# lorenlugosch/end-to-end-SLU

Hardware: AMD Instinct MI355X
Metric: utterances/sec (train step, 3 s @16 kHz, B=64) (higher is better)
Workload: dtype f32 (trainable stages: exact fp32 MFMA; convolutions and GRU contractions of FROZEN stages: bf16x3 = every fp32 operand split EXACTLY into 3 bf16 terms (3 x 8 = 24 significand bits, fp32's exponent range), 6 bf16 MFMA products per fp32 product (only terms below 2^-24 |a b| dropped), fp32 accumulatio; 1 GPU; experiments/no_unfreezing.cfg SLU train step (frozen SincNet/conv/biGRU encoder in train mode + intent biGRU trained): fwd + 3-slot CE + bwd + grad all-reduce + Adam; batch_per_gpu=64, global_batch=64, samples_per_utterance=48000, parallelism=dp1, encoder_lookahead_batches=20

## Files before the change

end-to-end-slu_amd/csrc/slu_gru_bf16.hip:

```cpp
#include "slu_bf16.h"
#include <type_traits>

namespace slu {

__device__ __forceinline__ float bf_sigmoid(float x) {
  return __builtin_amdgcn_rcpf(1.0f + __builtin_amdgcn_exp2f(-1.4426950408889634f * x));
}
__device__ __forceinline__ float bf_tanh(float x) {
  return 1.0f - 2.0f * __builtin_amdgcn_rcpf(1.0f + __builtin_amdgcn_exp2f(2.8853900817779268f * x));
}

__device__ __forceinline__ void lds_barrier() { asm volatile("s_waitcnt lgkmcnt(0)\n\ts_barrier" ::: "memory"); }

__device__ __forceinline__ float mul_rnd(float a, float b) {
#pragma clang fp contract(off)
  return a * b;
}
__device__ __forceinline__ float add_rnd(float a, float b) {
#pragma clang fp contract(off)
  return a + b;
}

struct GruBfParams {
  const float* gx;
  const unsigned short* xp; long long x_plane;
  const uint4* wih; const float* b_ih;
  const float* w_hh[2];
  const float* b_hh[2];
  float* out;
  float* reserve;
  unsigned short* planes; long long plane;
  const unsigned* keep;
  float keep_scale;
  int T, B, D;
};

template <int H, int NS, int KI, int EPI>
struct GruLds {
  static constexpr int ROWB = H * 2;
  static constexpr int GXROW = 3 * H + 8;
  static constexpr int OROW = H + 4;
  static constexpr int PROWB = H * 2 + 16;
  static constexpr int HBUF = 2 * NS * 16 * ROWB;
  static constexpr int BIAS = KI > 0 ? 2 * 3 * H * 4 : 0;
  static constexpr int GXS = KI > 0 ? 0 : 2 * 16 * GXROW * 4;
  static constexpr int OST = EPI == 1 ? 2 * NS * 16 * PROWB : 2 * 16 * OROW * 4;
  static constexpr int BYTES = HBUF + BIAS + GXS + OST;
};

template <int H, int NS, int KI, int EPI, bool REV>
__device__ __forceinline__ void gru_bf_fwd_body(const GruBfParams& p) {
  constexpr int NW = H / 16;
  constexpr int KC = H / 32;
  constexpr int SLOTS = H / 8;
  constexpr bool BIAS_LDS = KI > 0;
  typedef Split<NS> SP;
  typedef GruLds<H, NS, KI, EPI> LD;
  constexpr int ROWB = LD::ROWB, GXROW = LD::GXROW, OROW = LD::OROW, PROWB = LD::PROWB;
  extern __shared__ __attribute__((aligned(16))) unsigned char smem[];
  unsigned char* const hbuf = smem;
  float* const bias_s = reinterpret_cast<float*>(smem + LD::HBUF);
  float* const gxs = reinterpret_cast<float*>(smem + LD::HBUF + LD::BIAS);
  unsigned char* const ost = smem + LD::HBUF + LD::BIAS + LD::GXS;
  const int tid = threadIdx.x, lane = tid & 63;
  const int w = __builtin_amdgcn_readfirstlane(tid >> 6);
  const int i = lane & 15, kg = lane >> 4;
  constexpr int dir = REV ? 1 : 0;
  const int b0 = blockIdx.x * 16;
  const int u0 = w * 16 + kg * 4;
  const int T = p.T, B = p.B, D = p.D;
  const int seq = b0 + i;
  const int seqc = seq < B ? seq : B - 1;

  if constexpr (NS == 2) f16_denorm_flush();

  uint4 wb[3][KC][NS];
  {
    const float* __restrict__ W = p.w_hh[dir];
#pragma unroll
    for (int g = 0; g < 3; ++g)
#pragma unroll
      for (int c = 0; c < KC; ++c) {
        const float* src = W + (size_t)(g * H + w * 16 + i) * H + c * 32 + kg * 8;
        const float4 lo = *reinterpret_cast<const float4*>(src), hi = *reinterpret_cast<const float4*>(src + 4);
        const float v[8] = {lo.x, lo.y, lo.z, lo.w, hi.x, hi.y, hi.z, hi.w};
        unsigned short s[8][NS];
#pragma unroll
        for (int e = 0; e < 8; ++e) split_terms<NS>(v[e], s[e]);
#pragma unroll
        for (int pl = 0; pl < NS; ++pl) {
          uint4 o;
          o.x = s[0][pl] | ((unsigned)s[1][pl] << 16); o.y = s[2][pl] | ((unsigned)s[3][pl] << 16);
          o.z = s[4][pl] | ((unsigned)s[5][pl] << 16); o.w = s[6][pl] | ((unsigned)s[7][pl] << 16);
          wb[g][c][pl] = o;
        }
      }
  }
  float bh[3][4];
  if constexpr (BIAS_LDS) {
    for (int x = tid; x < 3 * H; x += H * 4) {
      bias_s[x] = p.b_hh[dir][x];
      bias_s[3 * H + x] = p.b_ih[(size_t)dir * 3 * H + x];
    }
  } else {
#pragma unroll
    for (int g = 0; g < 3; ++g) {
      const float4 v = *reinterpret_cast<const float4*>(p.b_hh[dir] + g * H + u0);
      bh[g][0] = v.x; bh[g][1] = v.y; bh[g][2] = v.z; bh[g][3] = v.w;
    }
  }
  constexpr int KIA = KI > 0 ? KI : 1;
  uint4 wi[3][KIA][NS];
  if constexpr (KI > 0) {
    const int NTI = p.D * 3 * NW;
#pragma unroll
    for (int g = 0; g < 3; ++g)
#pragma unroll
      for (int c = 0; c < KI; ++c)
#pragma unroll
        for (int pl = 0; pl < NS; ++pl)
          wi[g][c][pl] = p.wih[(size_t)pl * KI * NTI * 64 + ((size_t)c * NTI + dir * 3 * NW + g * NW + w) * 64 + lane];
  }
  auto xproj = [&](const uint4 (&xa)[KIA][NS], float (&o)[3][4]) {
    f32x4 ax[SP::NACC][3];
#pragma unroll
    for (int a = 0; a < SP::NACC; ++a)
#pragma unroll
      for (int g = 0; g < 3; ++g) ax[a][g] = f32x4{0.f, 0.f, 0.f, 0.f};
#pragma unroll
    for (int c = 0; c < KIA; ++c)
#pragma unroll
      for (int q = 0; q < SP::NPAIR; ++q)
#pragma unroll
        for (int g = 0; g < 3; ++g)
          ax[SP::ACC(q)][g] = mfma_split<NS>(wi[g][c][SP::PB(q)], xa[c][SP::PA(q)], ax[SP::ACC(q)][g]);
#pragma unroll
    for (int g = 0; g < 3; ++g) {
      const f32x4 v = split_result<NS>(ax[0][g], ax[SP::NACC - 1][g]);
      const float4 bi = *reinterpret_cast<const float4*>(&bias_s[BIAS_LDS ? 3 * H + g * H + u0 : 0]);
      o[g][0] = v[0] + bi.x; o[g][1] = v[1] + bi.y; o[g][2] = v[2] + bi.z; o[g][3] = v[3] + bi.w;
    }
  };
  auto xload = [&](int t_, uint4 (&xa)[KIA][NS]) {
    const unsigned short* base = p.xp + ((size_t)t_ * B + seqc) * (32 * KIA) + kg * 8;
#pragma unroll
    for (int c = 0; c < KIA; ++c)
#pragma unroll
      for (int pl = 0; pl < NS; ++pl)
        xa[c][pl] = *reinterpret_cast<const uint4*>(base + (size_t)pl * p.x_plane + c * 32);
  };

  constexpr int RW = 16 / NW;
  constexpr int GLR = 3 * H / 4;
  auto gx_g = [&](int j) { const int f = j * 64 + lane; return min(b0 + RW * w + f / GLR, B - 1) * D * 3 * H + dir * 3 * H + (f % GLR) * 4; };
  auto gx_s = [&](int j) { const int f = j * 64 + lane; return (RW * w + f / GLR) * GXROW + (f % GLR) * 4; };
  const int gx_g0 = gx_g(0), gx_g1 = gx_g(1), gx_g2 = gx_g(2);
  const int gx_s0 = gx_s(0), gx_s1 = gx_s(1), gx_s2 = gx_s(2);
  const size_t gx_ts = (size_t)B * D * 3 * H, out_ts = (size_t)B * D * H;
#define SLU_GX_REQUEST(t_, a, b, c)                                                         \
  do {                                                                                      \
    const float* gp__ = p.gx + (size_t)(t_) * gx_ts;                                        \
    a = *reinterpret_cast<const float4*>(gp__ + gx_g0);                                     \
    b = *reinterpret_cast<const float4*>(gp__ + gx_g1);                                     \
    c = *reinterpret_cast<const float4*>(gp__ + gx_g2);                                     \
  } while (0)
#define SLU_GX_STAGE(buf, a, b, c)                                                          \
  do {                                                                                      \
    float* gs__ = gxs + (buf) * (16 * GXROW);                                               \
    *reinterpret_cast<float4*>(gs__ + gx_s0) = a;                                           \
    *reinterpret_cast<float4*>(gs__ + gx_s1) = b;                                           \
    *reinterpret_cast<float4*>(gs__ + gx_s2) = c;                                           \
  } while (0)
  const int orow = RW * w + lane / (H / 4), oc16 = lane % (H / 4);
  const bool orow_ok = b0 + orow < B;
  const int o_goff = (b0 + orow) * D * H + dir * H + oc16 * 4;

  int a_off[KC];
#pragma unroll
  for (int c = 0; c < KC; ++c) a_off[c] = i * ROWB + (((c * 4 + kg) ^ i) & (SLOTS - 1)) * 16;
  const int h_off = i * ROWB + ((((u0 >> 3) ^ i) & (SLOTS - 1)) * 16) + (u0 & 7) * 2;
  const int gs_off = i * GXROW + u0;
  const int os_off = i * OROW + u0;
  const int ps_off = i * PROWB + u0 * 2;
  const int kw_off = seqc * ((D * H) >> 5) + ((dir * H + u0) >> 5);
  const int kw_sh = (dir * H + u0) & 31;
  const size_t kw_ts = (size_t)B * ((D * H) >> 5);
  const bool drop = EPI > 0 && p.keep != nullptr;

  for (int x = tid; x < 2 * NS * 16 * ROWB / 4; x += H * 4) reinterpret_cast<unsigned*>(hbuf)[x] = 0u;
  float hprev[4] = {0.f, 0.f, 0.f, 0.f};
  float gcur[3][4];
  unsigned kcur = 0;
  {
    const int t0 = dir ? T - 1 : 0;
    if constexpr (KI > 0) {
      __syncthreads();
      uint4 xa0[KIA][NS];
      xload(t0, xa0);
      xproj(xa0, gcur);
    } else {
      float4 ga, gb, gc;
      SLU_GX_REQUEST(t0, ga, gb, gc);
      SLU_GX_STAGE(0, ga, gb, gc);
    }
    if (drop) kcur = p.keep[(size_t)t0 * kw_ts + kw_off];
  }
  float held[4] = {0.f, 0.f, 0.f, 0.f};
  int pend_t = -1;
  int pend_buf = 0;
  auto flush = [&]() {
    if (pend_t < 0) return;
    if constexpr (EPI == 1) {
      constexpr int LPR = H / 8;
      constexpr int NCH = NS * 16 * LPR / 64;
      for (int c = w; c < NCH; c += NW) {
        const int f = c * 64 + lane, pl = f / (16 * LPR), r = (f / LPR) % 16, c16 = f % LPR;
        if (b0 + r < B) {
          const uint4 v = *reinterpret_cast<const uint4*>(ost + ((pend_buf * NS + pl) * 16 + r) * PROWB + c16 * 16);
          *reinterpret_cast<uint4*>(p.planes + (size_t)pl * p.plane + (size_t)pend_t * out_ts + (b0 + r) * D * H + dir * H + c16 * 8) = v;
        }
      }
    } else {
      if (orow_ok) {
        const float4 v = *reinterpret_cast<const float4*>(reinterpret_cast<const float*>(ost) + (pend_buf * 16 + orow) * OROW + oc16 * 4);
        *reinterpret_cast<float4*>(p.out + (size_t)pend_t * out_ts + o_goff) = v;
      }
    }
  };
  __syncthreads();
  __builtin_amdgcn_s_waitcnt(0x0F70);

  auto step = [&](auto cur_c, const int s) {
    constexpr int cur = decltype(cur_c)::value;
    const int t = dir ? T - 1 - s : s;
    const int tn = (s + 1 < T) ? (dir ? t - 1 : t + 1) : t;

    if constexpr (BIAS_LDS) {
#pragma unroll
      for (int g = 0; g < 3; ++g) {
        const float4 v = *reinterpret_cast<const float4*>(&bias_s[g * H + u0]);
        bh[g][0] = v.x; bh[g][1] = v.y; bh[g][2] = v.z; bh[g][3] = v.w;
      }
    }
    if constexpr (KI == 0) {
#pragma unroll
      for (int g = 0; g < 3; ++g) {
        const float4 v = *reinterpret_cast<const float4*>(gxs + cur * (16 * GXROW) + gs_off + g * H);
        gcur[g][0] = v.x; gcur[g][1] = v.y; gcur[g][2] = v.z; gcur[g][3] = v.w;
      }
    }
    f32x4 accs[SP::NACC][3];
#pragma unroll
    for (int a = 0; a < SP::NACC; ++a)
#pragma unroll
      for (int g = 0; g < 3; ++g) accs[a][g] = f32x4{0.f, 0.f, 0.f, 0.f};
    float gn[4];
#pragma unroll
    for (int r = 0; r < 4; ++r) {
      accs[0][0][r] = gcur[0][r] + bh[0][r];
      accs[0][1][r] = gcur[1][r] + bh[1][r];
      accs[0][2][r] = bh[2][r];
      gn[r] = gcur[2][r];
    }
    const unsigned kbits = kcur >> kw_sh;

    float gnext[3][4];
    float4 gl0 = make_float4(0.f, 0.f, 0.f, 0.f), gl1 = gl0, gl2 = gl0;
    uint4 xan[KIA][NS];
    if constexpr (KI > 0) xload(tn, xan);
    else SLU_GX_REQUEST(tn, gl0, gl1, gl2);
    unsigned knext = 0;
    if (drop) knext = p.keep[(size_t)tn * kw_ts + kw_off];
    flush();

    const unsigned char* hc = hbuf + cur * (NS * 16 * ROWB);
    float hn[4];
#pragma unroll
    for (int c = 0; c < KC; ++c) {
      uint4 fa[NS];
#pragma unroll
      for (int pl = 0; pl < NS; ++pl) fa[pl] = *reinterpret_cast<const uint4*>(hc + pl * (16 * ROWB) + a_off[c]);
#pragma unroll
      for (int q = 0; q < SP::NPAIR; ++q)
#pragma unroll
        for (int g = 0; g < 3; ++g)
          accs[SP::ACC(q)][g] = mfma_split<NS>(wb[g][c][SP::PB(q)], fa[SP::PA(q)], accs[SP::ACC(q)][g]);
    }
    f32x4 acc[3];
#pragma unroll
    for (int g = 0; g < 3; ++g) acc[g] = split_result<NS>(accs[0][g], accs[SP::NACC - 1][g]);

#pragma unroll
    for (int r = 0; r < 4; ++r) {
      const float rr = bf_sigmoid(acc[0][r]);
      const float zz = bf_sigmoid(acc[1][r]);
      const float nn = bf_tanh(gn[r] + rr * acc[2][r]);
      hn[r] = nn + zz * (hprev[r] - nn);
    }
    {
      unsigned char* __restrict__ hnext = hbuf + (cur ^ 1) * (NS * 16 * ROWB);
      if constexpr (NS == 2) {
        unsigned hi01, lo01, hi23, lo23;
        split_f16x2_pair_flush(hn[0], hn[1], hi01, lo01);
        split_f16x2_pair_flush(hn[2], hn[3], hi23, lo23);
        *reinterpret_cast<uint2*>(hnext + h_off) = make_uint2(hi01, hi23);
        *reinterpret_cast<uint2*>(hnext + 16 * ROWB + h_off) = make_uint2(lo01, lo23);
      } else if constexpr (NS == 3) {
        unsigned w01[3], w23[3];
        split_bf16x3_pair(hn[0], hn[1], w01);
        split_bf16x3_pair(hn[2], hn[3], w23);
#pragma unroll
        for (int pl = 0; pl < 3; ++pl)
          *reinterpret_cast<uint2*>(hnext + pl * (16 * ROWB) + h_off) = make_uint2(w01[pl], w23[pl]);
      } else {
        unsigned short sp[4][NS];
#pragma unroll
        for (int r = 0; r < 4; ++r) split_terms<NS>(hn[r], sp[r]);
#pragma unroll
        for (int pl = 0; pl < NS; ++pl)
          *reinterpret_cast<uint2*>(hnext + pl * (16 * ROWB) + h_off) =
              make_uint2(sp[0][pl] | ((unsigned)sp[1][pl] << 16), sp[2][pl] | ((unsigned)sp[3][pl] << 16));
      }
    }
    if constexpr (EPI == 0) {
      *reinterpret_cast<float4*>(reinterpret_cast<float*>(ost) + cur * (16 * OROW) + os_off) = make_float4(hn[0], hn[1], hn[2], hn[3]);
      pend_t = t; pend_buf = cur;
    } else {
      float m[4];
#pragma unroll
      for (int r = 0; r < 4; ++r)
        m[r] = drop ? mul_rnd(hn[r], ((kbits >> r) & 1u) ? p.keep_scale : 0.0f) : hn[r];
      const bool even = dir ? (t & 1) == 0 : cur == 0;
      const bool single = even && t == T - 1;
      const bool emit = dir ? even : (!even || single);
      pend_t = -1;
      if (!emit) {
#pragma unroll
        for (int r = 0; r < 4; ++r) held[r] = dir ? m[r] : add_rnd(0.0f, m[r]);
      } else {
        float v[4];
#pragma unroll
        for (int r = 0; r < 4; ++r) {
          const float first = dir ? add_rnd(0.0f, m[r]) : held[r];
          const float second = dir ? held[r] : m[r];
          v[r] = mul_rnd(add_rnd(first, second), 0.5f);
        }
        if (single) {
          asm volatile("" ::: "memory");
#pragma unroll
          for (int r = 0; r < 4; ++r) v[r] = add_rnd(0.0f, m[r]);
        }
        pend_t = t >> 1; pend_buf = cur;
        if constexpr (EPI == 2) {
          *reinterpret_cast<float4*>(reinterpret_cast<float*>(ost) + cur * (16 * OROW) + os_off) = make_float4(v[0], v[1], v[2], v[3]);
        } else if constexpr (NS == 2) {
          unsigned hi01, lo01, hi23, lo23;
          split_f16x2_pair_flush(v[0], v[1], hi01, lo01);
          split_f16x2_pair_flush(v[2], v[3], hi23, lo23);
          *reinterpret_cast<uint2*>(ost + ((cur * NS + 0) * 16) * PROWB + ps_off) = make_uint2(hi01, hi23);
          *reinterpret_cast<uint2*>(ost + ((cur * NS + 1) * 16) * PROWB + ps_off) = make_uint2(lo01, lo23);
        } else if constexpr (NS == 3) {
          unsigned w01[3], w23[3];
          split_bf16x3_pair(v[0], v[1], w01);
          split_bf16x3_pair(v[2], v[3], w23);
#pragma unroll
          for (int pl = 0; pl < 3; ++pl)
            *reinterpret_cast<uint2*>(ost + ((cur * NS + pl) * 16) * PROWB + ps_off) = make_uint2(w01[pl], w23[pl]);
        } else {
          unsigned short sp[4][NS];
#pragma unroll
          for (int r = 0; r < 4; ++r) split_terms<NS>(v[r], sp[r]);
#pragma unroll
          for (int pl = 0; pl < NS; ++pl)
            *reinterpret_cast<uint2*>(ost + ((cur * NS + pl) * 16) * PROWB + ps_off) =
                make_uint2(sp[0][pl] | ((unsigned)sp[1][pl] << 16), sp[2][pl] | ((unsigned)sp[3][pl] << 16));
        }
      }
    }
    if constexpr (KI > 0) {
      xproj(xan, gnext);
#pragma unroll
      for (int g = 0; g < 3; ++g)
#pragma unroll
        for (int r = 0; r < 4; ++r) gcur[g][r] = gnext[g][r];
    } else {
      SLU_GX_STAGE(cur ^ 1, gl0, gl1, gl2);
    }
#pragma unroll
    for (int r = 0; r < 4; ++r) hprev[r] = hn[r];
    kcur = knext;
    lds_barrier();
  };
  {
    int s = 0;
    for (; s + 1 < T; s += 2) {
      step(std::integral_constant<int, 0>{}, s);
      step(std::integral_constant<int, 1>{}, s + 1);
    }
    if (s < T) step(std::integral_constant<int, 0>{}, s);
  }
  flush();
#undef SLU_GX_REQUEST
#undef SLU_GX_STAGE
}

template <int H, int NS, int KI, int EPI>
__global__ void __launch_bounds__(H * 4)
gru_bf_fwd_kernel(const GruBfParams p) {
  if (blockIdx.y) gru_bf_fwd_body<H, NS, KI, EPI, true>(p);
  else gru_bf_fwd_body<H, NS, KI, EPI, false>(p);
}

template <int H, int NS, int EPI>
struct Gru2Lds {
  static constexpr int ROWB = H * 2;
  static constexpr int OROW = H + 4;
  static constexpr int PROWB = H * 2 + 16;
  static constexpr int HB = NS * 16 * ROWB;
  static constexpr int GXB = 16 * 3 * H * 4;
  static constexpr int KBB = 16 * (H / 32) * 4;
  static constexpr int OSB = EPI == 1 ? NS * 16 * PROWB : 16 * OROW * 4;
  static constexpr int HBUF = 0;
  static constexpr int GXR = HBUF + 2 * HB;
  static constexpr int KBR = GXR + 3 * GXB;
  static constexpr int BIAS = KBR + 3 * KBB;
  static constexpr int OST = BIAS + 3 * H * 4;
  static constexpr int HP = OST + 2 * OSB;
  static constexpr int HELD = HP + 2 * 16 * H * 4;
  static constexpr int BYTES = HELD + (EPI > 0 ? 2 * 16 * H * 4 : 0);
};

__device__ __forceinline__ void dma_b128(const void* base, unsigned voff, unsigned lds_addr) {
  asm volatile("s_mov_b32 m0, %2\n\ts_nop 0\n\tglobal_load_lds_dwordx4 %0, %1" :: "v"(voff), "s"(base), "s"(lds_addr) : "memory");
}
__device__ __forceinline__ void dma_b32(const void* base, unsigned voff, unsigned lds_addr) {
  asm volatile("s_mov_b32 m0, %2\n\ts_nop 0\n\tglobal_load_lds_dword %0, %1" :: "v"(voff), "s"(base), "s"(lds_addr) : "memory");
}

template <int H, int NS, int EPI>
__global__ void __launch_bounds__(H * 4)
gru_bf2_fwd_kernel(const GruBfParams p) {
  static_assert(H == 128, "two-tile recurrence: H = 128 (8 waves = two per SIMD, one keep-word DMA per chunk)");
  constexpr int NW = H / 16, KC = H / 32, SLOTS = H / 8;
  typedef Split<NS> SP;
  typedef Gru2Lds<H, NS, EPI> LD;
  constexpr int ROWB = LD::ROWB, OROW = LD::OROW, PROWB = LD::PROWB;
  constexpr int PCS = 3 * H / 4;
  extern __shared__ __attribute__((aligned(16))) unsigned char smem[];
  typedef __attribute__((address_space(3))) void* lptr_t;
  const unsigned lds0 = (unsigned)(size_t)(lptr_t)smem;
  float* const bias_s = reinterpret_cast<float*>(smem + LD::BIAS);
  const int tid = threadIdx.x, lane = tid & 63;
  const int w = __builtin_amdgcn_readfirstlane(tid >> 6);
  const int i = lane & 15, kg = lane >> 4;
  const int dir = blockIdx.y;
  const int b0 = blockIdx.x * 32;
  const int u0 = w * 16 + kg * 4;
  const int T = p.T, B = p.B, D = p.D;

  if constexpr (NS == 2) f16_denorm_flush();

  uint4 wb[3][KC][NS];
  {
    const float* __restrict__ W = p.w_hh[dir];
#pragma unroll
    for (int g = 0; g < 3; ++g)
#pragma unroll
      for (int c = 0; c < KC; ++c) {
        const float* src = W + (size_t)(g * H + w * 16 + i) * H + c * 32 + kg * 8;
        const float4 lo = *reinterpret_cast<const float4*>(src), hi = *reinterpret_cast<const float4*>(src + 4);
        const float v[8] = {lo.x, lo.y, lo.z, lo.w, hi.x, hi.y, hi.z, hi.w};
        unsigned short s[8][NS];
#pragma unroll
        for (int e = 0; e < 8; ++e) split_terms<NS>(v[e], s[e]);
#pragma unroll
        for (int pl = 0; pl < NS; ++pl) {
          uint4 o;
          o.x = s[0][pl] | ((unsigned)s[1][pl] << 16); o.y = s[2][pl] | ((unsigned)s[3][pl] << 16);
          o.z = s[4][pl] | ((unsigned)s[5][pl] << 16); o.w = s[6][pl] | ((unsigned)s[7][pl] << 16);
          wb[g][c][pl] = o;
        }
      }
  }
  for (int x = tid; x < 3 * H; x += H * 4) bias_s[x] = p.b_hh[dir][x];
  for (int x = tid; x < 2 * LD::HB / 4; x += H * 4) reinterpret_cast<unsigned*>(smem + LD::HBUF)[x] = 0u;
  __syncthreads();

  const bool drop = EPI > 0 && p.keep != nullptr;
  unsigned gv[2][3];
#pragma unroll
  for (int x = 0; x < 2; ++x)
#pragma unroll
    for (int j = 0; j < 3; ++j) {
      const int P = (3 * w + j) * 64 + lane, row = P / PCS, q = P % PCS;
      gv[x][j] = (unsigned)((min(b0 + 16 * x + row, B - 1) * D * 3 * H + dir * 3 * H) * 4 + (q ^ (row & 15)) * 16);
    }
  unsigned kv[2];
  const int KW = (D * H) >> 5;
#pragma unroll
  for (int x = 0; x < 2; ++x)
    kv[x] = drop ? (unsigned)((min(b0 + 16 * x + (lane >> 2), B - 1) * KW + dir * (H >> 5) + (lane & 3)) * 4) : (unsigned)(lane * 4);
  const void* const kbase = drop ? (const void*)p.keep : (const void*)p.gx;
  const size_t gx_ts = (size_t)B * D * 3 * H * 4, kw_ts = drop ? (size_t)B * KW * 4 : 0, out_ts = (size_t)B * D * H;
  const unsigned gx_m0 = lds0 + LD::GXR + 3 * w * 1024, kb_m0 = lds0 + LD::KBR;
  auto dma_chunk = [&](int x, int t_, int slot) {
    const char* gb = reinterpret_cast<const char*>(p.gx) + (size_t)t_ * gx_ts;
    const unsigned m = gx_m0 + slot * LD::GXB;
    const unsigned v0 = x ? gv[1][0] : gv[0][0], v1 = x ? gv[1][1] : gv[0][1], v2 = x ? gv[1][2] : gv[0][2];
    dma_b128(gb, v0, m);
    dma_b128(gb, v1, m + 1024);
    dma_b128(gb, v2, m + 2048);
    dma_b32(reinterpret_cast<const char*>(kbase) + (size_t)t_ * kw_ts, x ? kv[1] : kv[0], kb_m0 + slot * LD::KBB);
  };

  const int a_off0 = i * ROWB + ((kg ^ i) & (SLOTS - 1)) * 16;
  const int h_off = i * ROWB + ((((u0 >> 3) ^ i) & (SLOTS - 1)) * 16) + (u0 & 7) * 2;
  const int gs_off0 = (i * PCS + ((u0 >> 2) ^ i)) * 16;
  const int hp_off = (i * H + u0) * 4;
  const int kb_off = (i * (H >> 5) + (u0 >> 5)) * 4;
  const int kb_sh = u0 & 31;
  const int os_off = i * OROW + u0;
  const int ps_off = i * PROWB + u0 * 2;
  const int orow = (16 / NW) * w + lane / (H / 4), oc16 = lane % (H / 4);

  f32x4 accs[2][SP::NACC][3];
  float gn[2][4];
  unsigned kb[2] = {0u, 0u};
  int pend[2] = {-1, -1};
#pragma unroll
  for (int x = 0; x < 2; ++x) {
#pragma unroll
    for (int r = 0; r < 4; ++r) gn[x][r] = 0.f;
    *reinterpret_cast<float4*>(smem + LD::HP + x * (16 * H * 4) + hp_off) = make_float4(0.f, 0.f, 0.f, 0.f);
    if constexpr (EPI > 0) *reinterpret_cast<float4*>(smem + LD::HELD + x * (16 * H * 4) + hp_off) = make_float4(0.f, 0.f, 0.f, 0.f);
  }
#pragma unroll
  for (int x = 0; x < 2; ++x)
#pragma unroll
    for (int a = 0; a < SP::NACC; ++a)
#pragma unroll
      for (int g = 0; g < 3; ++g) accs[x][a][g] = f32x4{0.f, 0.f, 0.f, 0.f};

#define SLU_G2_M(X, slot)                                                                                              \
  do {                                                                                                                 \
    const unsigned char* gxc__ = smem + LD::GXR + (slot) * LD::GXB;                                                    \
    _Pragma("unroll") for (int g = 0; g < 3; ++g) {                                                                    \
      const float4 v = *reinterpret_cast<const float4*>(gxc__ + gs_off0 + g * (4 * H));                                \
      const float4 bb = *reinterpret_cast<const float4*>(&bias_s[g * H + u0]);                                         \
      _Pragma("unroll") for (int a = 0; a < SP::NACC; ++a) accs[X][a][g] = f32x4{0.f, 0.f, 0.f, 0.f};                  \
      if (g < 2) accs[X][0][g] = f32x4{v.x + bb.x, v.y + bb.y, v.z + bb.z, v.w + bb.w};                                \
      else { accs[X][0][g] = f32x4{bb.x, bb.y, bb.z, bb.w}; gn[X][0] = v.x; gn[X][1] = v.y; gn[X][2] = v.z; gn[X][3] = v.w; } \
    }                                                                                                                  \
    kb[X] = *reinterpret_cast<const unsigned*>(smem + LD::KBR + (slot) * LD::KBB + kb_off) >> kb_sh;                   \
    const unsigned char* hc__ = smem + LD::HBUF + (X) * LD::HB;                                                        \
    _Pragma("unroll") for (int c = 0; c < KC; ++c) {                                                                   \
      uint4 fa[NS];                                                                                                    \
      _Pragma("unroll") for (int pl = 0; pl < NS; ++pl) fa[pl] = *reinterpret_cast<const uint4*>(hc__ + pl * (16 * ROWB) + (a_off0 ^ (c * 64))); \
      _Pragma("unroll") for (int q = 0; q < SP::NPAIR; ++q)                                                            \
        _Pragma("unroll") for (int g = 0; g < 3; ++g)                                                                  \
          accs[X][SP::ACC(q)][g] = mfma_split<NS>(wb[g][c][SP::PB(q)], fa[SP::PA(q)], accs[X][SP::ACC(q)][g]);         \
    }                                                                                                                  \
  } while (0)

#define SLU_G2_G(X, t_)                                                                                                \
  do {                                                                                                                 \
    f32x4 acc[3];                                                                                                      \
    _Pragma("unroll") for (int g = 0; g < 3; ++g) acc[g] = split_result<NS>(accs[X][0][g], accs[X][SP::NACC - 1][g]);  \
    float hn[4];                                                                                                       \
    float4* const hp__ = reinterpret_cast<float4*>(smem + LD::HP + (X) * (16 * H * 4) + hp_off);                       \
    const float4 hpv = *hp__;                                                                                          \
    const float hprev[4] = {hpv.x, hpv.y, hpv.z, hpv.w};                                                               \
    _Pragma("unroll") for (int r = 0; r < 4; ++r) {                                                                    \
      const float rr = bf_sigmoid(acc[0][r]);                                                                          \
      const float zz = bf_sigmoid(acc[1][r]);                                                                          \
      const float nn = bf_tanh(gn[X][r] + rr * acc[2][r]);                                                             \
      hn[r] = nn + zz * (hprev[r] - nn);                                                                               \
    }                                                                                                                  \
    *hp__ = make_float4(hn[0], hn[1], hn[2], hn[3]);                                                                   \
    {                                                                                                                  \
      unsigned char* __restrict__ hx = smem + LD::HBUF + (X) * LD::HB;                                                 \
      if constexpr (NS == 2) {                                                                                         \
        unsigned hi01, lo01, hi23, lo23;                                                                               \
        split_f16x2_pair_flush(hn[0], hn[1], hi01, lo01);                                                              \
        split_f16x2_pair_flush(hn[2], hn[3], hi23, lo23);                                                              \
        *reinterpret_cast<uint2*>(hx + h_off) = make_uint2(hi01, hi23);                                                \
        *reinterpret_cast<uint2*>(hx + 16 * ROWB + h_off) = make_uint2(lo01, lo23);                                    \
      } else if constexpr (NS == 3) {                                                                                  \
        unsigned w01[3], w23[3];                                                                                       \
        split_bf16x3_pair(hn[0], hn[1], w01);                                                                          \
        split_bf16x3_pair(hn[2], hn[3], w23);                                                                          \
        _Pragma("unroll") for (int pl = 0; pl < 3; ++pl)                                                               \
          *reinterpret_cast<uint2*>(hx + pl * (16 * ROWB) + h_off) = make_uint2(w01[pl], w23[pl]);                     \
      } else {                                                                                                         \
        unsigned short sp[4][NS];                                                                                      \
        _Pragma("unroll") for (int r = 0; r < 4; ++r) split_terms<NS>(hn[r], sp[r]);                                   \
        _Pragma("unroll") for (int pl = 0; pl < NS; ++pl)                                                              \
          *reinterpret_cast<uint2*>(hx + pl * (16 * ROWB) + h_off) =                                                   \
              make_uint2(sp[0][pl] | ((unsigned)sp[1][pl] << 16), sp[2][pl] | ((unsigned)sp[3][pl] << 16));            \
      }                                                                                                                \
    }                                                                                                                  \
    unsigned char* const ox__ = smem + LD::OST + (X) * LD::OSB;                                                        \
    if constexpr (EPI == 0) {                                                                                          \
      *reinterpret_cast<float4*>(reinterpret_cast<float*>(ox__) + os_off) = make_float4(hn[0], hn[1], hn[2], hn[3]);   \
      pend[X] = (t_);                                                                                                  \
    } else {                                                                                                           \
      float m[4];                                                                                                      \
      _Pragma("unroll") for (int r = 0; r < 4; ++r)                                                                    \
        m[r] = drop ? __fmul_rn(hn[r], ((kb[X] >> r) & 1u) ? p.keep_scale : 0.0f) : hn[r];                             \
      const bool even = ((t_) & 1) == 0;                                                                               \
      const bool single = even && (t_) == T - 1;                                                                       \
      const bool emit = dir ? even : (!even || single);                                                                \
      pend[X] = -1;                                                                                                    \
      float4* const hl__ = reinterpret_cast<float4*>(smem + LD::HELD + (X) * (16 * H * 4) + hp_off);                   \
      if (!emit) {                                                                                                     \
        float hd[4];                                                                                                   \
        _Pragma("unroll") for (int r = 0; r < 4; ++r) hd[r] = dir ? m[r] : __fadd_rn(0.0f, m[r]);                      \
        *hl__ = make_float4(hd[0], hd[1], hd[2], hd[3]);                                                               \
      } else {                                                                                                         \
        const float4 hlv = *hl__;                                                                                      \
        const float held[4] = {hlv.x, hlv.y, hlv.z, hlv.w};                                                            \
        float v[4];                                                                                                    \
        _Pragma("unroll") for (int r = 0; r < 4; ++r) {                                                                \
          const float first = dir ? __fadd_rn(0.0f, m[r]) : held[r];                                                   \
          const float second = dir ? held[r] : m[r];                                                                   \
          v[r] = single ? __fadd_rn(0.0f, m[r]) : __fmul_rn(__fadd_rn(first, second), 0.5f);                           \
        }                                                                                                              \
        pend[X] = (t_) >> 1;                                                                                           \
        if constexpr (EPI == 2) {                                                                                      \
          *reinterpret_cast<float4*>(reinterpret_cast<float*>(ox__) + os_off) = make_float4(v[0], v[1], v[2], v[3]);   \
        } else if constexpr (NS == 2) {                                                                                \
          unsigned hi01, lo01, hi23, lo23;                                                                             \
          split_f16x2_pair_flush(v[0], v[1], hi01, lo01);                                                              \
          split_f16x2_pair_flush(v[2], v[3], hi23, lo23);                                                              \
          *reinterpret_cast<uint2*>(ox__ + ps_off) = make_uint2(hi01, hi23);                                           \
          *reinterpret_cast<uint2*>(ox__ + 16 * PROWB + ps_off) = make_uint2(lo01, lo23);                              \
        } else if constexpr (NS == 3) {                                                                                \
          unsigned w01[3], w23[3];                                                                                     \
          split_bf16x3_pair(v[0], v[1], w01);                                                                          \
          split_bf16x3_pair(v[2], v[3], w23);                                                                          \
          _Pragma("unroll") for (int pl = 0; pl < 3; ++pl)                                                             \
            *reinterpret_cast<uint2*>(ox__ + (pl * 16) * PROWB + ps_off) = make_uint2(w01[pl], w23[pl]);               \
        } else {                                                                                                       \
          unsigned short sp[4][NS];                                                                                    \
          _Pragma("unroll") for (int r = 0; r < 4; ++r) split_terms<NS>(v[r], sp[r]);                                  \
          _Pragma("unroll") for (int pl = 0; pl < NS; ++pl)                                                            \
            *reinterpret_cast<uint2*>(ox__ + (pl * 16) * PROWB + ps_off) =                                             \
                make_uint2(sp[0][pl] | ((unsigned)sp[1][pl] << 16), sp[2][pl] | ((unsigned)sp[3][pl] << 16));          \
        }                                                                                                              \
      }                                                                                                                \
    }                                                                                                                  \
  } while (0)

#define SLU_G2_FLUSH(X)                                                                                                \
  do {                                                                                                                 \
    if (pend[X] >= 0) {                                                                                                \
      const unsigned char* ox__ = smem + LD::OST + (X) * LD::OSB;                                                      \
      if constexpr (EPI == 1) {                                                                                        \
        const int r = (w & 3) * 4 + (lane >> 4), c16 = lane & 15;                                                      \
        unsigned short* const gp__ = p.planes + (size_t)pend[X] * out_ts + (size_t)((b0 + 16 * (X) + r) * D * H + dir * H + c16 * 8); \
        const bool ok__ = b0 + 16 * (X) + r < B;                                                                       \
        if (w < NS * 4) {                                                                                              \
          const int pl = w >> 2;                                                                                       \
          const uint4 v = *reinterpret_cast<const uint4*>(ox__ + (pl * 16 + r) * PROWB + c16 * 16);                    \
          if (ok__) *reinterpret_cast<uint4*>(gp__ + (size_t)pl * p.plane) = v;                                        \
        }                                                                                                              \
        if (w + 8 < NS * 4) {                                                                                          \
          const int pl = (w >> 2) + 2;                                                                                 \
          const uint4 v = *reinterpret_cast<const uint4*>(ox__ + (pl * 16 + r) * PROWB + c16 * 16);                    \
          if (ok__) *reinterpret_cast<uint4*>(gp__ + (size_t)pl * p.plane) = v;                                        \
        }                                                                                                              \
      } else {                                                                                                         \
        const float4 v = *reinterpret_cast<const float4*>(reinterpret_cast<const float*>(ox__) + orow * OROW + oc16 * 4); \
        if (b0 + 16 * (X) + orow < B)                                                                                  \
          *reinterpret_cast<float4*>(p.out + (size_t)pend[X] * out_ts + (b0 + 16 * (X) + orow) * D * H + dir * H + oc16 * 4) = v; \
      }                                                                                                                \
    }                                                                                                                  \
  } while (0)

#define SLU_G2_PHASE(X, doM, doG, tg, tn)                                                                              \
  do {                                                                                                                 \
    SLU_G2_FLUSH(X);                                                                                                   \
    dma_chunk(X, tn, sl == 0 ? 2 : sl - 1);                                                                            \
    if constexpr (doM) SLU_G2_M(X, sl);                   \
    if constexpr (doG) SLU_G2_G(1 - (X), tg);                                                                          \
    asm volatile("s_waitcnt vmcnt(4)" ::: "memory");                                                                   \
    lds_barrier();                                                                                                     \
    sl = sl == 2 ? 0 : sl + 1;                                                                                         \
  } while (0)

  auto tt = [&](int s_) { const int c = s_ < T - 1 ? s_ : T - 1; return dir ? T - 1 - c : c; };
  dma_chunk(0, tt(0), 0);
  dma_chunk(1, tt(0), 1);
  asm volatile("s_waitcnt vmcnt(0)" ::: "memory");
  __syncthreads();

  int sl = 0;
  SLU_G2_PHASE(0, true, false, 0, tt(1));
  for (int s = 0; s + 1 < T; ++s) {
    SLU_G2_PHASE(1, true, true, tt(s), tt(s + 1));
    SLU_G2_PHASE(0, true, true, tt(s), tt(s + 2));
  }
  SLU_G2_PHASE(1, true, true, tt(T - 1), tt(T - 1));
  SLU_G2_PHASE(0, false, true, tt(T - 1), tt(T - 1));
  SLU_G2_FLUSH(1);
  asm volatile("s_waitcnt vmcnt(0)" ::: "memory");
#undef SLU_G2_PHASE
#undef SLU_G2_FLUSH
#undef SLU_G2_G
#undef SLU_G2_M
}

template <int H, int NS>
__global__ void __launch_bounds__(H * 4)
gru_bf_fwd_rs_kernel(const GruBfParams p) {
  constexpr int NW = H / 16, KC = H / 32, ROWB = H * 2, SLOTS = H / 8;
  typedef Split<NS> SP;
  __shared__ __attribute__((aligned(16))) unsigned char hbuf[2][NS][16 * ROWB];
  const int tid = threadIdx.x, lane = tid & 63;
  const int w = __builtin_amdgcn_readfirstlane(tid >> 6);
  const int i = lane & 15, kg = lane >> 4;
  const int dir = blockIdx.y;
  const int b0 = blockIdx.x * 16;
  const int j = w * 16 + i;
  const int T = p.T, B = p.B, D = p.D;

  uint4 wb[3][KC][NS];
  {
    const float* __restrict__ W = p.w_hh[dir];
#pragma unroll
    for (int g = 0; g < 3; ++g)
#pragma unroll
      for (int c = 0; c < KC; ++c) {
        const float* src = W + (size_t)(g * H + j) * H + c * 32 + kg * 8;
        const float4 lo = *reinterpret_cast<const float4*>(src), hi = *reinterpret_cast<const float4*>(src + 4);
        const float v[8] = {lo.x, lo.y, lo.z, lo.w, hi.x, hi.y, hi.z, hi.w};
        unsigned short s[8][NS];
#pragma unroll
        for (int e = 0; e < 8; ++e) split_terms<NS>(v[e], s[e]);
#pragma unroll
        for (int pl = 0; pl < NS; ++pl) {
          uint4 o;
          o.x = s[0][pl] | ((unsigned)s[1][pl] << 16); o.y = s[2][pl] | ((unsigned)s[3][pl] << 16);
          o.z = s[4][pl] | ((unsigned)s[5][pl] << 16); o.w = s[6][pl] | ((unsigned)s[7][pl] << 16);
          wb[g][c][pl] = o;
        }
      }
  }
  const float bhr = p.b_hh[dir][j], bhz = p.b_hh[dir][H + j], bhn = p.b_hh[dir][2 * H + j];
  for (int x = tid; x < 2 * NS * 16 * ROWB / 4; x += H * 4) reinterpret_cast<unsigned*>(&hbuf[0][0][0])[x] = 0u;
  float hprev[4] = {0.f, 0.f, 0.f, 0.f};
  int g_off[4], o_off[4];
#pragma unroll
  for (int r = 0; r < 4; ++r) {
    const int b = b0 + 4 * kg + r;
    g_off[r] = (b < B ? b : 0) * D * 3 * H;
    o_off[r] = b < B ? b * D * H : -1;
  }
  const size_t gx_ts = (size_t)B * D * 3 * H, out_ts = (size_t)B * D * H;
  const float* __restrict__ gxd = p.gx + (size_t)dir * 3 * H + j;
  float* __restrict__ outd = p.out + (size_t)dir * H + j;
  int a_off[KC];
#pragma unroll
  for (int c = 0; c < KC; ++c) a_off[c] = i * ROWB + (((c * 4 + kg) ^ i) & (SLOTS - 1)) * 16;
  int h_off[4];
#pragma unroll
  for (int r = 0; r < 4; ++r) {
    const int row = 4 * kg + r;
    h_off[r] = row * ROWB + ((((j >> 3) ^ row) & (SLOTS - 1)) * 16) + (j & 7) * 2;
  }
  float gr[4], gz[4], gn[4];
  {
    const int t0 = dir ? T - 1 : 0;
#pragma unroll
    for (int r = 0; r < 4; ++r) {
      const float* g = gxd + (size_t)t0 * gx_ts + g_off[r];
      gr[r] = g[0]; gz[r] = g[H]; gn[r] = g[2 * H];
    }
  }
  __syncthreads();

  for (int s = 0; s < T; ++s) {
    const int t = dir ? T - 1 - s : s;
    const int cur = s & 1;
    float ngr[4], ngz[4], ngn[4];
    const int tn = (s + 1 < T) ? (dir ? t - 1 : t + 1) : t;
#pragma unroll
    for (int r = 0; r < 4; ++r) {
      const float* g = gxd + (size_t)tn * gx_ts + g_off[r];
      ngr[r] = g[0]; ngz[r] = g[H]; ngn[r] = g[2 * H];
    }
    f32x4 accs[SP::NACC][3];
#pragma unroll
    for (int a = 0; a < SP::NACC; ++a)
#pragma unroll
      for (int g = 0; g < 3; ++g) accs[a][g] = f32x4{0.f, 0.f, 0.f, 0.f};
#pragma unroll
    for (int c = 0; c < KC; ++c) {
      uint4 fa[NS];
#pragma unroll
      for (int pl = 0; pl < NS; ++pl) fa[pl] = *reinterpret_cast<const uint4*>(&hbuf[cur][pl][a_off[c]]);
#pragma unroll
      for (int q = 0; q < SP::NPAIR; ++q)
#pragma unroll
        for (int g = 0; g < 3; ++g)
          accs[SP::ACC(q)][g] = mfma_split<NS>(fa[SP::PA(q)], wb[g][c][SP::PB(q)], accs[SP::ACC(q)][g]);
    }
    f32x4 acc[3];
#pragma unroll
    for (int g = 0; g < 3; ++g) acc[g] = split_result<NS>(accs[0][g], accs[SP::NACC - 1][g]);

    float hn[4], rr[4], zz[4], nn[4], qq[4];
#pragma unroll
    for (int r = 0; r < 4; ++r) {
      rr[r] = bf_sigmoid(gr[r] + (acc[0][r] + bhr));
      zz[r] = bf_sigmoid(gz[r] + (acc[1][r] + bhz));
      qq[r] = acc[2][r] + bhn;
      nn[r] = bf_tanh(gn[r] + rr[r] * qq[r]);
      hn[r] = (1.0f - zz[r]) * nn[r] + zz[r] * hprev[r];
    }
    {
      float4* __restrict__ rs = reinterpret_cast<float4*>(
          p.reserve + ((((size_t)dir * T + t) * gridDim.x + blockIdx.x) * NW + w) * (5 * 256)) + lane;
      rs[0 * 64] = make_float4(rr[0], rr[1], rr[2], rr[3]);
      rs[1 * 64] = make_float4(zz[0], zz[1], zz[2], zz[3]);
      rs[2 * 64] = make_float4(nn[0], nn[1], nn[2], nn[3]);
      rs[3 * 64] = make_float4(qq[0], qq[1], qq[2], qq[3]);
      rs[4 * 64] = make_float4(hprev[0], hprev[1], hprev[2], hprev[3]);
    }
    unsigned char* __restrict__ hnext = &hbuf[cur ^ 1][0][0];
#pragma unroll
    for (int r = 0; r < 4; ++r) {
      unsigned short sp[NS];
      split_terms<NS>(hn[r], sp);
#pragma unroll
      for (int pl = 0; pl < NS; ++pl) *reinterpret_cast<unsigned short*>(hnext + pl * (16 * ROWB) + h_off[r]) = sp[pl];
      if (o_off[r] >= 0) outd[(size_t)t * out_ts + o_off[r]] = hn[r];
    }
#pragma unroll
    for (int r = 0; r < 4; ++r) { hprev[r] = hn[r]; gr[r] = ngr[r]; gz[r] = ngz[r]; gn[r] = ngn[r]; }
    __syncthreads();
  }
}

template <int H, int NS, int KI, int EPI>
static void gru_bf_launch(dim3 grid, hipStream_t st, const GruBfParams& p) {
  constexpr int lds = GruLds<H, NS, KI, EPI>::BYTES;
  static bool raised = false;
  if (lds > 64 * 1024 && !raised) {
    (void)hipFuncSetAttribute((const void*)gru_bf_fwd_kernel<H, NS, KI, EPI>, hipFuncAttributeMaxDynamicSharedMemorySize, lds);
    raised = true;
  }
  hipLaunchKernelGGL((gru_bf_fwd_kernel<H, NS, KI, EPI>), grid, dim3(H * 4), lds, st, p);
}

template <int H, int NS, int EPI>
static void gru_bf2_launch(hipStream_t st, const GruBfParams& p) {
  constexpr int lds = Gru2Lds<H, NS, EPI>::BYTES;
  static bool raised = false;
  if (lds > 64 * 1024 && !raised) {
    (void)hipFuncSetAttribute((const void*)gru_bf2_fwd_kernel<H, NS, EPI>, hipFuncAttributeMaxDynamicSharedMemorySize, lds);
    raised = true;
  }
  hipLaunchKernelGGL((gru_bf2_fwd_kernel<H, NS, EPI>), dim3((unsigned)cdiv(p.B, 32), (unsigned)p.D), dim3(H * 4), lds, st, p);
}

template <int H, int EPI>
static int gru_bf_dispatch(int nsplit, int ki, int seq_tiles, dim3 grid, hipStream_t st, const GruBfParams& p) {
  if (seq_tiles == 2) {
    if constexpr (H == 128) {
      if (nsplit == 3) gru_bf2_launch<128, 3, EPI>(st, p);
      else if (nsplit == 2) gru_bf2_launch<128, 2, EPI>(st, p);
      else gru_bf2_launch<128, 1, EPI>(st, p);
    }
    SLU_CHECK_LAUNCH("gru_bf2_fwd_kernel");
    return SLU_OK;
  }
  if (ki > 0) {
    if constexpr (H == 128) {
      if (nsplit == 3) {
        if (ki == 1) gru_bf_launch<128, 3, 1, EPI>(grid, st, p); else gru_bf_launch<128, 3, 2, EPI>(grid, st, p);
      } else {
        if (ki == 1) gru_bf_launch<128, 2, 1, EPI>(grid, st, p); else gru_bf_launch<128, 2, 2, EPI>(grid, st, p);
      }
    }
  } else if (nsplit == 3) {
    gru_bf_launch<H, 3, 0, EPI>(grid, st, p);
  } else if (nsplit == 2) {
    gru_bf_launch<H, 2, 0, EPI>(grid, st, p);
  } else {
    gru_bf_launch<H, 1, 0, EPI>(grid, st, p);
  }
  SLU_CHECK_LAUNCH("gru_bf_fwd_kernel");
  return SLU_OK;
}

}

using namespace slu;

static int gru_bf_common(const char* who, GruBfParams& p, const float* gx, const float* w_hh_fwd, const float* w_hh_rev,
                         const float* b_hh_fwd, const float* b_hh_rev, const void* x_planes, int64_t x_plane_stride,
                         int64_t K, const void* w_ih_packed, const float* b_ih, int64_t T, int64_t B, int64_t H, int64_t D,
                         int nsplit, bool has_reserve, int seq_tiles) {
  SLU_REQUIRE((gx || x_planes) && w_hh_fwd && b_hh_fwd, "%s: null pointer", who);
  SLU_REQUIRE(seq_tiles >= 0 && seq_tiles <= 2, "%s: seq_tiles must be 0 / 1 (one 16-sequence tile per workgroup) or 2", who);
  if (seq_tiles == 2 && !(H == 128 && gx && !x_planes && !has_reserve && B * D * 3 * H < (1LL << 30)))
    SLU_FAIL(SLU_ERR_UNSUPPORTED, "%s: two sequence tiles per workgroup are instantiated for H = 128, gx input (no fused "
             "projection), no reserve, B * D * 3H < 2^30 (got H %lld, B %lld)", who, (long long)H, (long long)B);
  const bool fused = x_planes != nullptr;
  if (fused) {
    SLU_REQUIRE(!gx && w_ih_packed && b_ih && !has_reserve, "%s: the fused input projection takes x_planes, "
                "w_ih_packed and b_ih instead of gx, and no reserve (frozen layers only)", who);
    if (!((nsplit == 2 || nsplit == 3) && H == 128 && K >= 1 && K <= 64))
      SLU_FAIL(SLU_ERR_UNSUPPORTED, "%s: the fused input projection is instantiated for f16x2 / bf16x3 (nsplit 2 / 3), "
               "H = 128 and at most 64 input channels (got nsplit %d, H %lld, K %lld)", who, nsplit, (long long)H, (long long)K);
    SLU_REQUIRE(x_plane_stride >= T * B * (cdiv(K, 32) * 32) && ((uintptr_t)x_planes & 15) == 0 && (x_plane_stride & 7) == 0,
                "%s: x plane stride / alignment", who);
  }
  SLU_REQUIRE(D == 1 || (D == 2 && w_hh_rev && b_hh_rev), "%s: D must be 1 or 2 (with reverse weights)", who);
  SLU_REQUIRE(T > 0 && B > 0, "%s: non-positive T or B", who);
  SLU_REQUIRE(nsplit >= 1 && nsplit <= 3, "%s: nsplit must be 1 (bf16), 2 (f16x2) or 3 (bf16x3)", who);
  if (H != 64 && H != 128)
    SLU_FAIL(SLU_ERR_UNSUPPORTED, "%s: hidden size %lld not instantiated (64, 128)", who, (long long)H);
  SLU_REQUIRE(cdiv(B, 16) <= 65535 && B * D * 3 * H < (1LL << 31), "%s: B too large", who);
  SLU_REQUIRE(!gx || ((uintptr_t)gx & 15) == 0, "%s: gx must be 16-byte aligned", who);
  SLU_REQUIRE(((uintptr_t)b_hh_fwd & 15) == 0 && ((uintptr_t)b_hh_rev & 15) == 0, "%s: biases must be 16-byte aligned", who);
  p.xp = (const unsigned short*)x_planes; p.x_plane = x_plane_stride; p.wih = (const uint4*)w_ih_packed; p.b_ih = b_ih;
  p.gx = gx; p.w_hh[0] = w_hh_fwd; p.w_hh[1] = w_hh_rev; p.b_hh[0] = b_hh_fwd; p.b_hh[1] = b_hh_rev;
  p.out = nullptr; p.reserve = nullptr; p.planes = nullptr; p.plane = 0; p.keep = nullptr; p.keep_scale = 1.0f;
  p.T = (int)T; p.B = (int)B; p.D = (int)D;
  return SLU_OK;
}

extern "C" int slu_gru_seq_fwd_bf16(const float* gx, const float* w_hh_fwd, const float* w_hh_rev,
                                    const float* b_hh_fwd, const float* b_hh_rev, float* out, float* reserve,
                                    const void* x_planes, int64_t x_plane_stride, int64_t K, const void* w_ih_packed,
                                    const float* b_ih, int64_t T, int64_t B, int64_t H, int64_t D, int nsplit,
                                    int seq_tiles, void* stream) {
  SLU_REQUIRE(out, "slu_gru_seq_fwd_bf16: null pointer");
  GruBfParams p;
  int rc = gru_bf_common("slu_gru_seq_fwd_bf16", p, gx, w_hh_fwd, w_hh_rev, b_hh_fwd, b_hh_rev, x_planes, x_plane_stride, K,
                         w_ih_packed, b_ih, T, B, H, D, nsplit, reserve != nullptr, seq_tiles);
  if (rc) return rc;
  p.out = out; p.reserve = reserve;
  dim3 grid((unsigned)cdiv(B, 16), (unsigned)D);
  hipStream_t st = (hipStream_t)stream;
  if (reserve) {
#define SLU_RS(H_, NS_) hipLaunchKernelGGL((gru_bf_fwd_rs_kernel<H_, NS_>), grid, dim3(H_ * 4), 0, st, p)
    if (H == 128) { if (nsplit == 3) SLU_RS(128, 3); else if (nsplit == 2) SLU_RS(128, 2); else SLU_RS(128, 1); }
    else { if (nsplit == 3) SLU_RS(64, 3); else if (nsplit == 2) SLU_RS(64, 2); else SLU_RS(64, 1); }
#undef SLU_RS
    SLU_CHECK_LAUNCH("gru_bf_fwd_rs_kernel");
    return SLU_OK;
  }
  SLU_REQUIRE(((uintptr_t)out & 15) == 0, "slu_gru_seq_fwd_bf16: out must be 16-byte aligned");
  const int ki = x_planes ? (K <= 32 ? 1 : 2) : 0;
  return H == 128 ? gru_bf_dispatch<128, 0>(nsplit, ki, seq_tiles, grid, st, p) : gru_bf_dispatch<64, 0>(nsplit, ki, seq_tiles, grid, st, p);
}

extern "C" int slu_gru_seq_fwd_pool_bf16(const float* gx, const float* w_hh_fwd, const float* w_hh_rev,
                                         const float* b_hh_fwd, const float* b_hh_rev, float* out_pooled,
                                         void* out_planes, int64_t out_plane_stride, const uint32_t* keep_bits, float p_drop,
                                         const void* x_planes, int64_t x_plane_stride, int64_t K, const void* w_ih_packed,
                                         const float* b_ih, int64_t T, int64_t B, int64_t H, int64_t D, int nsplit,
                                         int seq_tiles, void* stream) {
  SLU_REQUIRE((out_pooled != nullptr) != (out_planes != nullptr),
              "slu_gru_seq_fwd_pool_bf16: exactly one of out_pooled and out_planes");
  SLU_REQUIRE(p_drop >= 0.0f && p_drop < 1.0f && (keep_bits || p_drop == 0.0f),
              "slu_gru_seq_fwd_pool_bf16: dropout p in [0, 1), with keep_bits when p > 0");
  GruBfParams p;
  int rc = gru_bf_common("slu_gru_seq_fwd_pool_bf16", p, gx, w_hh_fwd, w_hh_rev, b_hh_fwd, b_hh_rev, x_planes,
                         x_plane_stride, K, w_ih_packed, b_ih, T, B, H, D, nsplit, false, seq_tiles);
  if (rc) return rc;
  if ((D * H) % 32 != 0)
    SLU_FAIL(SLU_ERR_UNSUPPORTED, "slu_gru_seq_fwd_pool_bf16: D * H must be a multiple of 32 (got %lld)", (long long)(D * H));
  const int64_t T_out = cdiv(T, 2);
  if (out_planes)
    SLU_REQUIRE(out_plane_stride >= T_out * B * D * H && ((uintptr_t)out_planes & 7) == 0 && (out_plane_stride & 3) == 0,
                "slu_gru_seq_fwd_pool_bf16: plane stride / alignment");
  else
    SLU_REQUIRE(((uintptr_t)out_pooled & 15) == 0, "slu_gru_seq_fwd_pool_bf16: out_pooled must be 16-byte aligned");
  p.out = out_pooled; p.planes = (unsigned short*)out_planes; p.plane = out_plane_stride;
  p.keep = p_drop > 0.0f ? keep_bits : nullptr; p.keep_scale = 1.0f / (1.0f - p_drop);
  dim3 grid((unsigned)cdiv(B, 16), (unsigned)D);
  hipStream_t st = (hipStream_t)stream;
  const int ki = x_planes ? (K <= 32 ? 1 : 2) : 0;
  if (out_planes)
    return H == 128 ? gru_bf_dispatch<128, 1>(nsplit, ki, seq_tiles, grid, st, p) : gru_bf_dispatch<64, 1>(nsplit, ki, seq_tiles, grid, st, p);
  return H == 128 ? gru_bf_dispatch<128, 2>(nsplit, ki, seq_tiles, grid, st, p) : gru_bf_dispatch<64, 2>(nsplit, ki, seq_tiles, grid, st, p);
}
```

Baseline: 376,300 utterances/s.

## Stage input-projection weight planes and x tiles in LDS for bf16x3 GRU

For the fused-input-projection bf16x3 GRU kernel, this moves the lower two weight split-planes from registers into LDS and loads them per chunk. Input activations are fetched cooperatively, one wave per plane and chunk, two steps ahead into a double-buffered LDS tile instead of each wave loading every plane. The output staging buffer is cut to a single buffer, with an extra barrier in the tail case, to make room in LDS. The aim is lower VGPR pressure and fewer redundant global loads, which could raise occupancy or shorten the per-step critical path. The cost is more LDS traffic and LDS footprint in the serial recurrence, plus a possible hazard from the single output buffer.

Result: no change. 377,300 utterances/s (median of 3 runs) (+0.3%).

```diff
diff --git a/end-to-end-slu_amd/csrc/slu_gru_bf16.hip b/end-to-end-slu_amd/csrc/slu_gru_bf16.hip
--- a/end-to-end-slu_amd/csrc/slu_gru_bf16.hip
+++ b/end-to-end-slu_amd/csrc/slu_gru_bf16.hip
@@ -35,6 +35,9 @@
   int T, B, D;
 };
 
+#ifndef SLU_GRU_WIH_LDS_PLANES
+#define SLU_GRU_WIH_LDS_PLANES 2
+#endif
 template <int H, int NS, int KI, int EPI>
 struct GruLds {
   static constexpr int ROWB = H * 2;
@@ -44,8 +47,12 @@
   static constexpr int HBUF = 2 * NS * 16 * ROWB;
   static constexpr int BIAS = KI > 0 ? 2 * 3 * H * 4 : 0;
   static constexpr int GXS = KI > 0 ? 0 : 2 * 16 * GXROW * 4;
-  static constexpr int OST = EPI == 1 ? 2 * NS * 16 * PROWB : 2 * 16 * OROW * 4;
-  static constexpr int BYTES = HBUF + BIAS + GXS + OST;
+  static constexpr int WL = (KI > 0 && NS == 3) ? SLU_GRU_WIH_LDS_PLANES : 0;
+  static constexpr int WIH = WL * (H / 16) * 3 * KI * 64 * 16;
+  static constexpr int XS = WL > 0 ? 2 * KI * NS * 64 * 16 : 0;
+  static constexpr int OBUFS = (WL > 0 && EPI == 1) ? 1 : 2;
+  static constexpr int OST = EPI == 1 ? OBUFS * NS * 16 * PROWB : 2 * 16 * OROW * 4;
+  static constexpr int BYTES = HBUF + BIAS + GXS + OST + WIH + XS;
 };
 
 template <int H, int NS, int KI, int EPI, bool REV>
@@ -62,6 +69,8 @@
   float* const bias_s = reinterpret_cast<float*>(smem + LD::HBUF);
   float* const gxs = reinterpret_cast<float*>(smem + LD::HBUF + LD::BIAS);
   unsigned char* const ost = smem + LD::HBUF + LD::BIAS + LD::GXS;
+  const uint4* const wis = reinterpret_cast<const uint4*>(smem + LD::HBUF + LD::BIAS + LD::GXS + LD::OST);
+  uint4* const xs = reinterpret_cast<uint4*>(smem + LD::HBUF + LD::BIAS + LD::GXS + LD::OST + LD::WIH);
   const int tid = threadIdx.x, lane = tid & 63;
   const int w = __builtin_amdgcn_readfirstlane(tid >> 6);
   const int i = lane & 15, kg = lane >> 4;
@@ -110,7 +119,9 @@
     }
   }
   constexpr int KIA = KI > 0 ? KI : 1;
-  uint4 wi[3][KIA][NS];
+  constexpr int WL = LD::WL, WR = NS - WL;
+  uint4 wi[3][KIA][WR];
+  auto wis_at = [&](int pl, int g, int c) { return (((pl - WR) * NW + w) * 3 + g) * KIA + c; };
   if constexpr (KI > 0) {
     const int NTI = p.D * 3 * NW;
 #pragma unroll
@@ -118,8 +129,13 @@
 #pragma unroll
       for (int c = 0; c < KI; ++c)
 #pragma unroll
-        for (int pl = 0; pl < NS; ++pl)
-          wi[g][c][pl] = p.wih[(size_t)pl * KI * NTI * 64 + ((size_t)c * NTI + dir * 3 * NW + g * NW + w) * 64 + lane];
+        for (int pl = 0; pl < NS; ++pl) {
+          const uint4 v = p.wih[(size_t)pl * KI * NTI * 64 + ((size_t)c * NTI + dir * 3 * NW + g * NW + w) * 64 + lane];
+          if constexpr (WL > 0) {
+            if (pl >= WR) { const_cast<uint4*>(wis)[wis_at(pl, g, c) * 64 + lane] = v; continue; }
+          }
+          wi[g][c][pl < WR ? pl : 0] = v;
+        }
   }
   auto xproj = [&](const uint4 (&xa)[KIA][NS], float (&o)[3][4]) {
     f32x4 ax[SP::NACC][3];
@@ -128,12 +144,23 @@
 #pragma unroll
       for (int g = 0; g < 3; ++g) ax[a][g] = f32x4{0.f, 0.f, 0.f, 0.f};
 #pragma unroll
-    for (int c = 0; c < KIA; ++c)
+    for (int c = 0; c < KIA; ++c) {
+      uint4 wl[3][WL > 0 ? WL : 1];
+      if constexpr (WL > 0) {
+#pragma unroll
+        for (int g = 0; g < 3; ++g)
+#pragma unroll
+          for (int pl = WR; pl < NS; ++pl) wl[g][pl - WR] = wis[wis_at(pl, g, c) * 64 + lane];
+      }
 #pragma unroll
       for (int q = 0; q < SP::NPAIR; ++q)
 #pragma unroll
-        for (int g = 0; g < 3; ++g)
-          ax[SP::ACC(q)][g] = mfma_split<NS>(wi[g][c][SP::PB(q)], xa[c][SP::PA(q)], ax[SP::ACC(q)][g]);
+        for (int g = 0; g < 3; ++g) {
+          const int pb = SP::PB(q);
+          ax[SP::ACC(q)][g] = mfma_split<NS>(pb < WR ? wi[g][c][pb < WR ? pb : 0] : wl[g][pb >= WR ? pb - WR : 0],
+                                             xa[c][SP::PA(q)], ax[SP::ACC(q)][g]);
+        }
+    }
 #pragma unroll
     for (int g = 0; g < 3; ++g) {
       const f32x4 v = split_result<NS>(ax[0][g], ax[SP::NACC - 1][g]);
@@ -148,6 +175,20 @@
 #pragma unroll
       for (int pl = 0; pl < NS; ++pl)
         xa[c][pl] = *reinterpret_cast<const uint4*>(base + (size_t)pl * p.x_plane + c * 32);
+  };
+
+  constexpr bool XSH = LD::XS > 0;
+  const bool xs_mine = XSH && w < KIA * NS;
+  const unsigned xl_off = (unsigned)(seqc * (32 * KIA) + kg * 8) * 2u;
+  auto xload1 = [&](int t_) {
+    const unsigned char* base = reinterpret_cast<const unsigned char*>(p.xp + (size_t)t_ * B * (32 * KIA) + (size_t)(w % NS) * p.x_plane + (w / NS) * 32);
+    return *reinterpret_cast<const uint4*>(base + xl_off);
+  };
+  auto xs_read = [&](int buf, uint4 (&xa)[KIA][NS]) {
+#pragma unroll
+    for (int c = 0; c < KIA; ++c)
+#pragma unroll
+      for (int pl = 0; pl < NS; ++pl) xa[c][pl] = xs[((buf * KIA + c) * NS + pl) * 64 + lane];
   };
 
   constexpr int RW = 16 / NW;
@@ -198,6 +239,10 @@
       uint4 xa0[KIA][NS];
       xload(t0, xa0);
       xproj(xa0, gcur);
+      if constexpr (XSH) {
+        const int t1 = T > 1 ? (dir ? T - 2 : 1) : t0;
+        if (xs_mine) xs[(KIA * NS + w) * 64 + lane] = xload1(t1);
+      }
     } else {
       float4 ga, gb, gc;
       SLU_GX_REQUEST(t0, ga, gb, gc);
@@ -214,10 +259,11 @@
       constexpr int LPR = H / 8;
       constexpr int NCH = NS * 16 * LPR / 64;
       for (int c = w; c < NCH; c += NW) {
-        const int f = c * 64 + lane, pl = f / (16 * LPR), r = (f / LPR) % 16, c16 = f % LPR;
+        const int f = c * 64 + lane, r = (f / LPR) % 16, c16 = f % LPR;
+        const int pl = c / (16 * LPR / 64);
         if (b0 + r < B) {
-          const uint4 v = *reinterpret_cast<const uint4*>(ost + ((pend_buf * NS + pl) * 16 + r) * PROWB + c16 * 16);
-          *reinterpret_cast<uint4*>(p.planes + (size_t)pl * p.plane + (size_t)pend_t * out_ts + (b0 + r) * D * H + dir * H + c16 * 8) = v;
+          const uint4 v = *reinterpret_cast<const uint4*>(ost + (((LD::OBUFS > 1 ? pend_buf : 0) * NS + pl) * 16 + r) * PROWB + c16 * 16);
+          *reinterpret_cast<uint4*>(p.planes + (size_t)pl * p.plane + (size_t)pend_t * out_ts + (unsigned)((b0 + r) * D * H + dir * H + c16 * 8)) = v;
         }
       }
     } else {
@@ -232,6 +278,7 @@
 
   auto step = [&](auto cur_c, const int s) {
     constexpr int cur = decltype(cur_c)::value;
+    constexpr int ocur = LD::OBUFS > 1 ? cur : 0;
     const int t = dir ? T - 1 - s : s;
     const int tn = (s + 1 < T) ? (dir ? t - 1 : t + 1) : t;
 
@@ -267,10 +314,14 @@
     float gnext[3][4];
     float4 gl0 = make_float4(0.f, 0.f, 0.f, 0.f), gl1 = gl0, gl2 = gl0;
     uint4 xan[KIA][NS];
-    if constexpr (KI > 0) xload(tn, xan);
+    uint4 xf = make_uint4(0u, 0u, 0u, 0u);
+    if constexpr (XSH) {
+      const int tn2 = (s + 2 < T) ? (dir ? t - 2 : t + 2) : t;
+      if (xs_mine) xf = xload1(tn2);
+    } else if constexpr (KI > 0) xload(tn, xan);
     else SLU_GX_REQUEST(tn, gl0, gl1, gl2);
     unsigned knext = 0;
-    if (drop) knext = p.keep[(size_t)tn * kw_ts + kw_off];
+    if (drop) knext = (p.keep + (size_t)tn * kw_ts)[(unsigned)kw_off];
     flush();
 
     const unsigned char* hc = hbuf + cur * (NS * 16 * ROWB);
@@ -347,6 +398,9 @@
         }
         if (single) {
           asm volatile("" ::: "memory");
+          if constexpr (EPI == 1 && LD::OBUFS == 1) {
+            if (!dir) lds_barrier();
+          }
 #pragma unroll
           for (int r = 0; r < 4; ++r) v[r] = add_rnd(0.0f, m[r]);
         }
@@ -357,27 +411,31 @@
           unsigned hi01, lo01, hi23, lo23;
           split_f16x2_pair_flush(v[0], v[1], hi01, lo01);
           split_f16x2_pair_flush(v[2], v[3], hi23, lo23);
-          *reinterpret_cast<uint2*>(ost + ((cur * NS + 0) * 16) * PROWB + ps_off) = make_uint2(hi01, hi23);
-          *reinterpret_cast<uint2*>(ost + ((cur * NS + 1) * 16) * PROWB + ps_off) = make_uint2(lo01, lo23);
+          *reinterpret_cast<uint2*>(ost + ((ocur * NS + 0) * 16) * PROWB + ps_off) = make_uint2(hi01, hi23);
+          *reinterpret_cast<uint2*>(ost + ((ocur * NS + 1) * 16) * PROWB + ps_off) = make_uint2(lo01, lo23);
         } else if constexpr (NS == 3) {
           unsigned w01[3], w23[3];
           split_bf16x3_pair(v[0], v[1], w01);
           split_bf16x3_pair(v[2], v[3], w23);
 #pragma unroll
           for (int pl = 0; pl < 3; ++pl)
-            *reinterpret_cast<uint2*>(ost + ((cur * NS + pl) * 16) * PROWB + ps_off) = make_uint2(w01[pl], w23[pl]);
+            *reinterpret_cast<uint2*>(ost + ((ocur * NS + pl) * 16) * PROWB + ps_off) = make_uint2(w01[pl], w23[pl]);
         } else {
           unsigned short sp[4][NS];
 #pragma unroll
           for (int r = 0; r < 4; ++r) split_terms<NS>(v[r], sp[r]);
 #pragma unroll
           for (int pl = 0; pl < NS; ++pl)
-            *reinterpret_cast<uint2*>(ost + ((cur * NS + pl) * 16) * PROWB + ps_off) =
+            *reinterpret_cast<uint2*>(ost + ((ocur * NS + pl) * 16) * PROWB + ps_off) =
                 make_uint2(sp[0][pl] | ((unsigned)sp[1][pl] << 16), sp[2][pl] | ((unsigned)sp[3][pl] << 16));
         }
       }
     }
     if constexpr (KI > 0) {
+      if constexpr (XSH) {
+        xs_read(cur ^ 1, xan);
+        if (xs_mine) xs[(cur * KIA * NS + w) * 64 + lane] = xf;
+      }
       xproj(xan, gnext);
 #pragma unroll
       for (int g = 0; g < 3; ++g)
```
